# mfkiwl/conan-slam

Measured on AMD Instinct MI355X. Metric: ekf_update_steps_per_sec, higher is better.
Workload: dtype f32

## Files before the change

### conan_slam_amd/_capi.py

```python
from __future__ import annotations

import ctypes as C
import os
import re

_HERE = os.path.dirname(os.path.abspath(__file__))
LIB_PATH = os.path.join(_HERE, "lib", "libcslam_hip.so")
HEADER_PATH = os.path.join(_HERE, "..", "include", "cslam.h")

OK, ERR_BAD_ARG, ERR_CAPACITY, ERR_HIP, ERR_NO_DEVICE, ERR_ALLOC = 0, 1, 2, 3, 4, 5
FACTOR_OK, FACTOR_FALLBACK, FACTOR_ZEROED, FACTOR_SKIPPED, FACTOR_BAD_IDF, FACTOR_INTERNAL = 0, 1, 2, 4, 8, 16
FACTOR_HEADING_SKIPPED = 32
F32, F64 = 0, 1
Q_LOWER_CHOL_GAIN, Q_PREDICT_NM4, Q_REF_EXACT, Q_TEXTBOOK = 1, 2, 3, 0
STAGE_GATHER, STAGE_FACTOR, STAGE_GAIN, STAGE_DOWNDATE, N_STAGES = 0, 1, 2, 3, 4
STAGE_NAMES = ["gather", "factor", "gain", "downdate"]


class CslamError(RuntimeError):
    def __init__(self, code: int, msg: str):
        super().__init__(f"cslam status {code}: {msg}")
        self.code = code


BATCH_MC_SYMBOLS = ("cslam_ekf_batch_predict_each", "cslam_ekf_batch_get_poses")

LANDMARK_SYMBOLS = ("cslam_ekf_get_landmarks", "cslam_ekf_batch_get_landmarks")
_PROTOTYPES = {
    "cslam_ekf_get_landmarks": [C.c_void_p, C.c_int, C.c_int, C.c_void_p, C.c_void_p, C.c_void_p],
    "cslam_ekf_batch_get_landmarks": [C.c_void_p, C.c_int, C.c_int, C.c_void_p, C.c_void_p, C.c_void_p],
    "cslam_sim_batch_create": [C.c_void_p, C.c_int, C.c_int, C.POINTER(C.c_longlong), C.c_int, C.POINTER(C.c_void_p)],
    "cslam_sim_batch_destroy": [C.c_void_p],
    "cslam_sim_batch_scan": [C.c_void_p, C.c_void_p, C.c_double, C.c_void_p, C.c_longlong, C.POINTER(C.c_int),
                             C.POINTER(C.c_int), C.POINTER(C.c_int)],
    "cslam_sim_batch_get_scan": [C.c_void_p, C.c_int, C.c_void_p, C.c_void_p, C.c_void_p, C.c_void_p],
    "cslam_sim_batch_get_table": [C.c_void_p, C.c_void_p],
    "cslam_sim_batch_set_table": [C.c_void_p, C.c_void_p],
    "cslam_ekf_batch_update_scan": [C.c_void_p, C.c_void_p, C.c_void_p],
    "cslam_ekf_batch_augment_scan": [C.c_void_p, C.c_void_p, C.c_void_p],
}
SIM_BATCH_SYMBOLS = tuple(k for k in _PROTOTYPES if "sim_batch" in k or k.endswith("_scan"))


def declared_symbols(header_path: str = HEADER_PATH):
    text = open(header_path).read()
    text = re.sub(r"/\*.*?\*/", "", text, flags=re.S)
    return sorted(set(re.findall(r"\b(cslam_[a-z0-9_]+)\s*\(", text)))


_lib = None
hip_runtime_path = None


# ... 45 lines not shown
```

### conan_slam_amd/csrc/cslam_ekf.hip

```cpp
#include <hip/hip_runtime.h>

#include <algorithm>
#include <atomic>
#include <cfloat>
#include <cmath>
#include <cstdint>
#include <cstdlib>
#include <new>
#include <string>
#include <thread>
#include <vector>

#include "cslam_common.hpp"
#include "device_owners.hpp"
#include "ekf_kernels.hpp"
#include "ekf_kernels_fast.hpp"
#include "ekf_landmark_kernels.hpp"
#include "ekf_lookahead.hpp"
#include "ekf_pgemm_limbs.hpp"
#include "ekf_pose_kernels.hpp"
#include "host_linalg.hpp"

namespace cslam
{
// ... 18 lines not shown
        }
        else
        {
            j.idf_out[i - 2 * j.m] = j.idf[i - 2 * j.m];
        }
    }
    return true;
}
__global__ void __launch_bounds__(128) ekf_la_wide_f32(LaWideArgs a)
{
    if (la_wide_snapshot(a.snap))
    {
        return;
    }
    ekf_la_wide_body<1, 0>(a);
}
__global__ void __launch_bounds__(128) ekf_la_wide_f32_k64(LaWideArgs a)
{
    if (la_wide_snapshot(a.snap))
    {
        return;
    }
    ekf_la_wide_body<1, 64>(a);
}
}

using namespace cslam;

namespace
{

std::atomic<int>& g_engines = ::cslam::live_engines();

constexpr int    kStagingSlots = 64;
constexpr size_t kLdsBudget    = 150 * 1024;

struct EkfBase
{
    virtual ~EkfBase() {}
    int         dtype    = CSLAM_F32;
    int         fuse_f64 = 1;
    int         pgemm_limbs_req = -1, limbs_kmin_req = -1;
    int         xcd_queues_req = -1;
    int         device   = 0;
    int         quirks   = CSLAM_Q_REF_EXACT;
    int         nmax     = 0;
    int         ncap     = 0;
    int         ldp      = 0;
    int         n        = 3;
    int         sync_mode = 1;
    int         seq_defer     = 1;
    int         lower         = 0;
    int         pipeline      = 0;
    int         pgemm_spare   = 16;
    int         gather_corr_wide = 1;
    int         pgemm_wgs     = 0;
    int         lookahead     = -1;
    Stream      stream_own, stream_b_own, stream_f_own;
    hipStream_t stream   = nullptr;
    hipStream_t stream_b = nullptr;
    long long   la_windows = 0;
    long long   stage_launches = 0;

    virtual int init()                                                                        = 0;
    virtual int set_state(const void* X, int n, const void* P, int ldp)                        = 0;
    virtual int get_state(void* X, void* P, int ldp)                                           = 0;
    virtual int get_x(void* X, int cap)                                                        = 0;
    virtual int get_landmarks(int first, int count, void* x, void* pll, void* pvl)             = 0;
    virtual int trace(double* tr)                                                              = 0;
    virtual int predict(double v, double swa, const void* Q, double wb, double dt)             = 0;
    virtual int update(const void* Z, int m, const void* R, const int* idf, int batch, bool on_device) = 0;
    virtual int augment(const void* Z, int q, const void* R)                                   = 0;
    virtual int observe_heading(double phi, int use)                                           = 0;
    virtual int associate(const void* Z, int m, const void* R, double g1, double g2, int* idf_out, int* kind) = 0;
    virtual int factor_status(int* flags, int clear)                                           = 0;
    virtual int set_profiling(int on)                                                          = 0;
    virtual int get_stage_times(double* ms, int* launches)                                     = 0;
    virtual int debug_last_update(void* PHT, void* S, void* G, void* W1, void* V, int* k)      = 0;
    virtual int set_deferred(int max_cols)                                                     = 0;
    virtual int do_flush()                                                                     = 0;
    virtual int resolve_predict()                                                              = 0;
    virtual void set_fuse_predict(int on)                                                      = 0;
    virtual int sync_all()                                                                     = 0;
    virtual int la_drain()                                                                     = 0;
};
// ... 164 lines not shown
        {
            CSLAM_HIP_TRY(hipFuncSetAttribute(reinterpret_cast<const void*>(&ekf_factor_mfma_f64<64>),
                                              hipFuncAttributeMaxDynamicSharedMemorySize, 160 * 1024));
            CSLAM_HIP_TRY(hipFuncSetAttribute(reinterpret_cast<const void*>(&ekf_factor_mfma_f64<32>),
                                              hipFuncAttributeMaxDynamicSharedMemorySize, 160 * 1024));
            CSLAM_HIP_TRY(hipFuncSetAttribute(reinterpret_cast<const void*>(&ekf_downdate_f64<4>),
                                              hipFuncAttributeMaxDynamicSharedMemorySize, 160 * 1024));
            CSLAM_HIP_TRY(hipFuncSetAttribute(reinterpret_cast<const void*>(&ekf_downdate_f64<2>),
                                              hipFuncAttributeMaxDynamicSharedMemorySize, 160 * 1024));
        }
        CSLAM_TRY(dTicket.alloc_zeroed(2, stream));
        if (const char* sv = getenv("CSLAM_LA_K64"))
        {
            la_k64 = atoi(sv) ? 1 : 0;
        }
        if (const char* sv = getenv("CSLAM_LA_WG_SIGNAL"))
        {
            la_wg_signal = atoi(sv) ? 1 : 0;
        }
        if (const char* sv = getenv("CSLAM_LA_HOLD_WIDE"))
        {
            la_hold_wide = atoi(sv) ? 1 : 0;
        }
        if (const char* sv = getenv("CSLAM_PSYM_NT"))
        {
            psym_nt = atoi(sv) ? 1 : 0;
        }
        rc = ensure_k(64);
        if (rc)
        {
            return rc;
        }
        rc = ensure_w(128);
        if (rc)
        {
            return rc;
        }
        rc = ensure_m(64);
        if (rc)
        {
            return rc;
        }
        CSLAM_HIP_TRY(hipStreamSynchronize(stream));
        return CSLAM_OK;
    }

// ... 18 lines not shown
        if (cols <= wcap)
        {
            return CSLAM_OK;
        }
        int rc = flush();
        if (rc || (rc = sync_all()))
        {
            return rc;
        }
        int neww = round_up(std::max(cols, 2 * wcap), 8);
        DevBuf<T>   w1, y;
        DevBuf<int> sign;
        if ((rc = w1.alloc_zeroed((size_t)2 * ldp * neww, stream)) || (rc = y.alloc((size_t)std::max(kcap, 8) * neww)) ||
            (rc = sign.alloc_zeroed((size_t)2 * neww + 2, stream)))
        {
            return rc;
        }
        dW1   = std::move(w1);
        ws.dY = std::move(y);
        dSign = std::move(sign);
        hd_cols[0] = hd_cols[1] = 0;
        wcap      = neww;
        wcur      = 0;
        last_slot = nullptr;
        return CSLAM_OK;
    }

    int sync_all() override
    {
        int rc = use_device();
        if (rc)
        {
            return rc;
        }
        CSLAM_HIP_TRY(hipStreamSynchronize(stream));
        if (stream_b != stream)
        {
            CSLAM_HIP_TRY(hipStreamSynchronize(stream_b));
        }
        if (stream_f)
        {
            CSLAM_HIP_TRY(hipStreamSynchronize(stream_f));
        }
        inflight_mask = 0;
        return CSLAM_OK;
    }
// ... 39 lines not shown
        {
            CSLAM_HIP_TRY(hipEventRecord(ev_a2b.get(), stream));
            CSLAM_HIP_TRY(hipStreamWaitEvent(stream_b, ev_a2b.get(), 0));
        }
        if (hd_cols[wcur] > 0)
        {
            if ((rc = launch_negcol_fix(W, kp, stream_b)))
            {
                return rc;
            }
        }
        if ((rc = prof_begin(CSLAM_STAGE_DOWNDATE, stream_b)) || (rc = launch_downdate(W, kp, stream_b)) ||
            (rc = prof_end(CSLAM_STAGE_DOWNDATE, stream_b)))
        {
            return rc;
        }
        if (stream_b != stream)
        {
            CSLAM_HIP_TRY(hipEventRecord(ev_pgemm.get(), stream_b));
            inflight_mask |= 1u << wcur;
        }
        wcur ^= 1;
        kp = 0;
        if ((rc = own_region(wcur)))
        {
            return rc;
        }
        if (hd_cols[wcur] > 0)
        {
            if (stream_b != stream)
            {
                CSLAM_HIP_TRY(hipMemsetAsync(dSign.get() + (size_t)wcur * wcap, 0, (size_t)wcap * sizeof(int), stream));
                CSLAM_HIP_TRY(hipMemsetAsync(dSign.get() + (size_t)2 * wcap + wcur, 0, sizeof(int), stream));
            }
            hd_cols[wcur] = 0;
        }
        return CSLAM_OK;
    }

    int ensure_tiles_morton(int tiles, hipStream_t stream)
    {
        if (tilesM_built == tiles)
        {
            return CSLAM_OK;
        }

// ... 151 lines not shown
        *dZ   = reinterpret_cast<const T*>(ds);
        *dIdf = reinterpret_cast<const int*>(ds + zb);
        return CSLAM_OK;
    }

    int set_state(const void* X, int nn, const void* P, int ldph) override
    {
        if (!X || !P || nn < 3 || nn > ncap || ((nn - 3) & 1) || ldph < nn)
        {
            return fail(CSLAM_ERR_BAD_ARG, "set_state: bad n=%d (cap %d) or ldp=%d", nn, ncap, ldph);
        }
        int rc = sync_all();
        if (rc)
        {
            return rc;
        }
        CSLAM_HIP_TRY(hipMemcpyAsync(dX.get(), X, (size_t)nn * sizeof(T), hipMemcpyHostToDevice, stream));
        CSLAM_HIP_TRY(hipMemcpy2DAsync(dP.get(), (size_t)ldp * sizeof(T), P, (size_t)ldph * sizeof(T),
                                       (size_t)nn * sizeof(T), (size_t)nn, hipMemcpyHostToDevice, stream));
        CSLAM_HIP_TRY(hipMemcpyAsync(dPv.get(), dP.get(), (size_t)3 * ldp * sizeof(T), hipMemcpyDeviceToDevice,
                                     stream));
        kp        = 0;
        wcur      = 0;
        last_slot = nullptr;
        hd_cols[0] = hd_cols[1] = 0;
        CSLAM_HIP_TRY(hipMemsetAsync(dSign.get(), 0, ((size_t)2 * wcap + 2) * sizeof(int), stream));
        CSLAM_HIP_TRY(hipMemsetAsync(ws.dPHT.get(), 0, (size_t)ldp * kcap * sizeof(T), stream));
        CSLAM_HIP_TRY(hipMemsetAsync(dW1.get(), 0, (size_t)2 * ldp * wcap * sizeof(T), stream));
        CSLAM_HIP_TRY(hipStreamSynchronize(stream));
        n = nn;
        return CSLAM_OK;
    }

    int get_state(void* X, void* P, int ldph) override
    {
        if (ldph < n && P)
        {
            return fail(CSLAM_ERR_BAD_ARG, "get_state: ldp=%d < n=%d", ldph, n);
        }
        int rc = use_device();
        if (rc)
        {
            return rc;
        }
        if (P && (rc = flush_wait()))
        {
// ... 711 lines not shown
    {
        DevBuf<T>   S, G, Gt, V, t, U, M, sub, xloc;
        DevBuf<int> idloc;
    };
    struct LaSet
    {
        Event          ev_fb;
        Event          ev_raw;
        FactorOut      fo[2];
        DevBuf<T>      XL, PvL, PH, PvLb, Dbb;
        DevBuf<T>      Y;
        DevBuf<LaModel<T>> model;
        DevBuf<unsigned>   done;
        DevBuf<long long>  stamps;
        DevBuf<int>        idf_keep;
        DevBuf<T>          z_keep;
    };
    struct LaHeld
    {
        bool       valid = false;
        bool       k64   = false;
        unsigned   grid  = 0;
        LaWideArgs wa;
    };
    LaHeld      la_held;
    int         la_hold_wide = 1;
    LaUpd       la_q[2];
    int         la_n = 0;
    LaSet       la;
    bool        la_ready = false;
    hipStream_t stream_f = nullptr;
    DevBuf<T>   la_WR;
    int         la_kpad  = 0;
    int         la_cus = 0;
    unsigned    la_target = 0;
    unsigned    la_seq    = 0;
    unsigned    la_sig_add = 0;
    int         la_k64 = 1;
    int         la_wg_signal = 0;

    int         la_fused   = 1;
    const T *dbgS = nullptr, *dbgGt = nullptr, *dbgV = nullptr;

    int la_ensure(int kp_cols)
    {
        constexpr int KM = 2 * kLaMaxObs;
        if (!la_ready)
        {
            int lo = 0, hi = 0;
            CSLAM_HIP_TRY(hipDeviceGetStreamPriorityRange(&lo, &hi));
            Stream sf;
            LaSet  nl;
            int    rc = sf.create_with_priority(hipStreamNonBlocking, hi);
            if (rc || (rc = nl.ev_fb.create(hipEventDisableTiming)) || (rc = nl.ev_raw.create(hipEventDisableTiming)))
            {
                return rc;
            }
            CSLAM_HIP_TRY(hipFuncSetAttribute(reinterpret_cast<const void*>(&ekf_la_chain_kernel<T, 32>),
                                              hipFuncAttributeMaxDynamicSharedMemorySize, (int)la_chain_lds<T>(32)));
            CSLAM_HIP_TRY(hipFuncSetAttribute(reinterpret_cast<const void*>(&ekf_la_chain_kernel<T, 64>),
                                              hipFuncAttributeMaxDynamicSharedMemorySize, (int)la_chain_lds<T>(64)));
            CSLAM_TRY(nl.done.alloc_zeroed_blocking(768));
// ... 19 lines not shown
            }
            if (const char* fv = getenv("CSLAM_LA_FUSED"))
            {
                la_fused = atoi(fv) ? 1 : 0;
            }
            stream_f_own = std::move(sf);
            stream_f     = stream_f_own.get();
            la           = std::move(nl);
            la_cus       = 1;
            la_target    = 0;
            la_seq       = 0;
            la_ready     = true;
        }
        if (kp_cols > la_kpad)
        {
            CSLAM_HIP_TRY(hipStreamSynchronize(stream));
            CSLAM_HIP_TRY(hipStreamSynchronize(stream_f));
            const int kpad = round_up(std::max(kp_cols, 128), 64);
            DevBuf<T> wr;
            CSLAM_TRY(wr.alloc((size_t)2 * KM * kpad));
            la_WR   = std::move(wr);
            la_kpad = kpad;
        }
        return CSLAM_OK;
    }

    bool la_eligible(int m) const
    {
        const int k = 2 * m;
        const bool on = lookahead > 0 || (lookahead < 0 && sizeof(T) == 4 && n >= 7000 && g_engines.load() == 1);
        return on && !sync_mode && !pipeline && profiling != 1 && k > 16 && k <= 2 * kLaMaxObs && gather_corr_wide &&
               fuse_predict && (sizeof(T) == 4 || fuse_f64) && defer_max >= k + (la_n ? 2 * la_q[0].m : k) &&
               wcap >= k + (la_n ? 2 * la_q[0].m : k) && seq.count == 0 && hd_cols[0] == 0 && hd_cols[1] == 0 && n > 3 &&
               kp_call_limit == 0;
    }

    int la_launch_held_wide(const LaSnapJob* job)
    {
        if (!la_held.valid)
        {
            return CSLAM_OK;
        }
        if constexpr (std::is_same<T, float>::value)
        {
            int rc = use_device();
            if (rc)
            {
                return rc;
            }
            if (g_engines.load() > 1)
            {
                CSLAM_HIP_TRY(hipStreamWaitEvent(stream, la.ev_fb.get(), 0));
            }
            LaWideArgs& wa = la_held.wa;
            unsigned    g  = la_held.grid;
            if (job != nullptr)
            {
                wa.snap = *job;
                g += 1;
            }
            if (la_held.k64)
            {
                hipLaunchKernelGGL(ekf_la_wide_f32_k64, dim3(g), dim3(128), 0, stream, wa);
            }
            else
            {
                hipLaunchKernelGGL(ekf_la_wide_f32, dim3(g), dim3(128), 0, stream, wa);
            }
            CSLAM_HIP_TRY(hipGetLastError());
        }
        la_held.valid = false;
        return CSLAM_OK;
    }

    int la_enqueue(const T* dZ, const int* dIdf, int m, const T* R, bool on_device)
    {
        if (on_device && la_n == 0)
        {
            int rc = la_held.valid ? ensure_m(m) : CSLAM_OK;
            if (rc)
            {
                return rc;
            }
            if constexpr (std::is_same<T, float>::value)
// ... 206 lines not shown
            return rc;
        }
        const T* Wp = wbase(wcur);
        LaRowsArgs<T> ra;
        ra.X     = dX.get();
        ra.Pv    = dPv.get();
        ra.ldp   = ldp;
        ra.n     = n;
        ra.idf_a = ua.dIdf;
        ra.ra    = ka;
        ra.idf_b = nu == 2 ? ub.dIdf : ua.dIdf;
        ra.rb    = kb;
        ra.Wp    = Wp;
        ra.ldw   = ldp;
        ra.kp    = kp;
        ra.kpad  = la_kpad;
        ra.XL    = la.XL.get();
        ra.PvL   = la.PvL.get();
        ra.WR    = la_WR.get();
        ra.flags = dFlags.get();
        ra.idf_b_keep = hold ? la.idf_keep.get() : (int*)nullptr;
        ra.Z_b        = ub.dZ;
        ra.Z_b_keep   = hold ? la.z_keep.get() : (T*)nullptr;
        hipLaunchKernelGGL(ekf_la_rows_kernel<T>, dim3(ka + kb), dim3(128), 0, stream, ra);
        LaPrepArgs<T> pa;
        pa.P       = dP.get();
        pa.ldp     = ldp;
        pa.n       = n;
        pa.lower   = lower;
        pa.X       = dX.get();
        pa.Pv      = dPv.get();
        pa.idf_a   = ua.dIdf;
        pa.idf_b   = nu == 2 ? ub.dIdf : ua.dIdf;
        pa.ra      = ka;
        pa.rb      = kb;
        pa.pp_a    = ua.pp;
        pa.XL      = la.XL.get();
        pa.PvL     = la.PvL.get();
        pa.WR      = la_WR.get();
        pa.kp      = kp;
        pa.kpad    = la_kpad;
        pa.sub_a   = la.fo[0].sub.get();
        pa.PH      = la.PH.get();
        pa.Dbb     = la.Dbb.get();
        pa.PvLb    = la.PvLb.get();
        pa.model_a = la.model.get();
        pa.xloc_a  = la.fo[0].xloc.get();
        pa.idloc   = la.fo[0].idloc.get();
        const int  k8f      = round_up(kp, 8);
        const bool pg_signal = !la_wg_signal && !safe && kp > 0 && seq.count == 0 && sizeof(T) == 4 && k8f <= 128 && lower && ldp < 32768 &&
                               !limbs_take(k8f) && stream_b == stream && hd_cols[wcur] == 0;
        pa.done    = pg_signal ? (unsigned*)nullptr : la.done.get();
        hipLaunchKernelGGL(ekf_la_blocks_kernel<T>, dim3(n_blocks), dim3(64), 0, stream, pa);
        CSLAM_HIP_TRY(hipGetLastError());
        if (safe)
        {
            CSLAM_HIP_TRY(hipEventRecord(la.ev_raw.get(), stream));
            CSLAM_HIP_TRY(hipStreamWaitEvent(stream_f, la.ev_raw.get(), 0));
            if ((rc = launch_chain()))
            {
                return rc;
            }
        }
        la_target += n_blocks;
        la_sig_add = pg_signal ? n_blocks : 0u;
        rc         = flush();
        if (la_sig_add != 0)
        {
            const unsigned add = la_sig_add;
            la_sig_add         = 0;
            hipLaunchKernelGGL(ekf_la_signal_kernel, dim3(1), dim3(64), 0, stream, la.done.get(), add);
        }
        if (rc)
        {
            return rc;
        }
// ... 23 lines not shown
                wa.mb      = nu == 2 ? ub.m : 0;
                wa.valid_a = ua.pp.valid;
                wa.valid_b = nu == 2 ? ub.pp.valid : 0;
                wa.w_a     = ua.pp.w;
                wa.w_b     = nu == 2 ? ub.pp.w : 0;
                wa.model_a = la.model.get();
                wa.model_b = la.model.get() + 1;
                wa.Gt_a    = la.fo[0].Gt.get();
                wa.u_a     = la.fo[0].U.get();
                wa.M_a     = la.fo[0].M.get();
                wa.sub_a   = la.fo[0].sub.get();
                wa.Gt_b    = la.fo[1].Gt.get();
                wa.u_b     = la.fo[1].U.get();
                wa.M_b     = la.fo[1].M.get();
                wa.sub_b   = la.fo[1].sub.get();
                wa.Y_b     = la.Y.get();
                wa.W1a     = wbase(wcur) + (size_t)kp * ldp;
                wa.W1b     = wa.W1a + (size_t)ka * ldp;
                wa.ldw     = ldp;
                wa.wv_out  = ws.dWv.get();
                wa.snap    = LaSnapJob{nullptr, nullptr, nullptr, nullptr, 0};
                la_held.wa    = wa;
                la_held.k64   = la_k64 && ua.m == 32 && (nu == 1 || ub.m == 32);
                la_held.grid  = (unsigned)(round_up(n, kTile) / 32);
                la_held.valid = true;
                if (!hold && (rc = la_launch_held_wide(nullptr)))
                {
                    return rc;
                }
                last_slot = nullptr;
                last_k    = 0;
                kp += ka + kb;
                sub_valid = false;
            }
        }
        if (!fused && ((rc = la_wide(ua, la.fo[0], la.ev_fb.get())) || (nu == 2 && (rc = la_wide(ub, la.fo[1],
                                                                                                 nullptr)))))
        {
            return rc;
        }
        pp = held;
        la_windows++;
        if (la.stamps.get() && la_windows == 300)
        {
            long long h[32];
            CSLAM_HIP_TRY(hipStreamSynchronize(stream));
// ... 783 lines not shown

int cslam_ekf_set_pgemm_workgroups(cslam_ekf_t h, int workgroups)
{
    CSLAM_NEED(h);
    if (workgroups < 0)
    {
        return fail(CSLAM_ERR_BAD_ARG, "set_pgemm_workgroups: negative");
    }
    B(h)->pgemm_wgs = workgroups;
    return CSLAM_OK;
}

int cslam_ekf_lookahead_windows(cslam_ekf_t h, long long* windows)
{
    CSLAM_NEED(h);
    if (!windows)
    {
        return fail(CSLAM_ERR_BAD_ARG, "lookahead_windows: null");
    }
    *windows = B(h)->la_windows;
    return CSLAM_OK;
}

int cslam_ekf_stage_launches(cslam_ekf_t h, long long* launches)
{
    CSLAM_NEED(h);
    if (!launches)
    {
        return fail(CSLAM_ERR_BAD_ARG, "stage_launches: null");
    }
    *launches = B(h)->stage_launches;
    return CSLAM_OK;
}

int cslam_ekf_get_streams(cslam_ekf_t h, void** chain_stream, void** pgemm_stream)
{
    CSLAM_NEED(h);
    if (chain_stream)
    {
        *chain_stream = reinterpret_cast<void*>(B(h)->stream);
    }
    if (pgemm_stream)
    {
        *pgemm_stream = reinterpret_cast<void*>(B(h)->stream_b);
    }
    return CSLAM_OK;
// ... 109 lines not shown
```

### conan_slam_amd/csrc/ekf_lookahead.hpp

```cpp
#pragma once

#include <hip/hip_runtime.h>

#include "ekf_kernels.hpp"
#include "ekf_kernels_fast.hpp"

namespace cslam
{

constexpr int kLaMaxObs = 32;

__device__ inline int la_row(const int* __restrict__ idf, int s, int n)
{
    return 3 + 2 * clamp_idf(idf[s >> 1], n) - 2 + (s & 1);
}

template <typename T>
struct LaRowsArgs
{
    const T* X;
    const T* Pv;
    int      ldp, n;
    const int* idf_a;
    int        ra;
// ... 316 lines not shown
            out[2 * tid + 1] = v1;
        }
        if (type == 2 && tid < 3)
        {
            a.PvLb[s * 3 + tid] = s_e3[tid];
        }
    }
    if (a.done == nullptr)
    {
        return;
    }
    __builtin_amdgcn_fence(__ATOMIC_RELEASE, "agent");
    __syncthreads();
    if (tid == 0)
    {
        atomicAdd(a.done + 16 * (blockIdx.x & 15u), 1u);
    }
}

template <typename T>
__global__ void __launch_bounds__(64) ekf_la_blocks_kernel(LaPrepArgs<T> a)
{
    ekf_la_blocks_body<T>(a);
}

template <typename T>
struct LaCarryArgs
{
    int n, m_a, m_b;
    const int* idf_b;
    PredictArgs<T> pp_b;
    const T *PH, *Dbb, *PvLb, *XLb;
    const LaModel<T>* model_a;
    const T *Gt_a, *u_a, *M_a, *sub_a;
    T*          sub_b;
    T*          xloc_b;
    LaModel<T>* model_b;
    T*          Y_b;
};

template <typename T>
inline size_t la_carry_lds()
{
    constexpr int KM = 2 * kLaMaxObs, LD = KM + 4, LB = 3 + KM + 1;
    return ((size_t)KM * LD + (size_t)(3 + KM) * LB + kLaMaxObs * 10 + (3 + KM) + 4 * KM + 3 * KM) * sizeof(T) + 64;
}
// ... 404 lines not shown
    const int *  idf_a, *idf_b;
    int          ma, mb;
    int          valid_a, valid_b, w_a, w_b;
    const LaModel<float>*model_a, *model_b;
    const float *Gt_a, *u_a, *M_a, *sub_a;
    const float *Gt_b, *u_b, *M_b, *sub_b, *Y_b;
    float *      W1a, *W1b;
    int          ldw;
    float*       wv_out;
    const unsigned* chain_done;
    unsigned        seq;
    unsigned long long timeout;
    int*            flags;
    long long*      stamps;
    long long*      wg_times;
    LaSnapJob       snap;
};

__device__ __forceinline__ int la_q_of(int t, int r, int lh)
{
    return 32 * t + (r & 3) + 8 * (r >> 2) + 4 * lh;
}

template <int PAIRS = 1, int KFIX = 0>
__device__ __forceinline__ void ekf_la_wide_body(const LaWideArgs& a)
{
    __shared__ __attribute__((aligned(16))) float s_G[2][4 * 1024];
    __shared__ __attribute__((aligned(16))) float s_Y[4 * 1024];
    __shared__ __attribute__((aligned(16))) float s_model[2][512];
    __shared__ __attribute__((aligned(16))) float s_u[2][256];
    __shared__ __attribute__((aligned(16))) float s_M[2][256];
    __shared__ int   s_fx[2][kLaMaxObs];
    __shared__ float s_sum_all[PAIRS][4][32];
    const int tid = threadIdx.x, wave = __builtin_amdgcn_readfirstlane(tid >> 6), lane = tid & 63, lj = lane & 31, lh = lane >> 5;
    const int wv = wave & 1, pr = wave >> 1;
    float (*s_sum)[32] = s_sum_all[pr];
    const int row0 = (blockIdx.x * PAIRS + pr) * 32;
    const int row  = row0 + lj;
    const int rowc = row < a.n ? row : a.n - 1;
    const int ka = KFIX ? KFIX : 2 * a.ma, kb = KFIX ? KFIX : 2 * a.mb;
    int       stamp_i = 0;
    auto      stamp   = [&]() {
        if (a.stamps != nullptr && blockIdx.x == (gridDim.x >> 1) && tid == 0)
        {
            a.stamps[stamp_i++] = (long long)__builtin_amdgcn_s_memrealtime();
        }
    };
    stamp();
    if constexpr (PAIRS == 2)
// ... 183 lines not shown
    };
    auto store_w1 = [&](float* W, int k, bool last) {
#pragma unroll
        for (int r = 0; r < 16; r++)
        {
            const int c = la_q_of(wv, r, lh);
            if (c < k)
            {
                if (row < 3)
                {
                    if (last)
                    {
                        a.wv_out[(size_t)row * k + c] = w1[r];
                    }
                    W[(size_t)c * a.ldw + row] = 0.f;
                }
                else
                {
                    W[(size_t)c * a.ldw + row] = w1[r];
                }
            }
        }
    };
    using U0 = std::integral_constant<int, 0>;
    using U1 = std::integral_constant<int, 1>;

    if (a.valid_a && row >= 3 && row - 3 < a.w_a)
    {
        float o0, o1, o2;
        predict_stripe_col<float>(s_model[0][0], s_model[0][1], pv0, pv1, pv2, &o0, &o1, &o2);
        pv0 = o0, pv1 = o1, pv2 = o2;
    }
    build_own(U0{}, ka, a.sub_a);
    share();
    stamp();
    gain(U0{}, ka);
    stamp();
    store_w1(a.W1a, ka, a.nu == 1);
    const float* pred_last = s_model[0];
    if (a.nu == 2)
    {
        __syncthreads();
#pragma unroll
        for (int r = 0; r < 16; r++)
        {
            own[r] = (row >= 3) ? w1[r] : 0.f;
        }
        share();
        const float xs = s_sum[0][lj], xm0 = s_sum[1][lj], xm1 = s_sum[2][lj], xm2 = s_sum[3][lj];
        if (row >= 3)
        {
            x += xs;
            pv0 -= xm0, pv1 -= xm1, pv2 -= xm2;
        }
        stamp();
        if (a.valid_b && row >= 3 && row - 3 < a.w_b)
        {
            float o0, o1, o2;
            predict_stripe_col<float>(s_model[1][0], s_model[1][1], pv0, pv1, pv2, &o0, &o1, &o2);
            pv0 = o0, pv1 = o1, pv2 = o2;
        }
// ... 24 lines not shown
                    c0 = __builtin_amdgcn_mfma_f32_32x32x2f32(y[i], full[i], c0, 0, 0, 0);
                }
            }
            if (row >= 3)
            {
#pragma unroll
                for (int r = 0; r < 16; r++)
                {
                    own[r] -= c0[r] + c1[r];
                }
            }
        }
        stamp();
        __syncthreads();
        dma(a.Gt_b, kb * kb, s_G[1]);
        xch = s_G[0] + pr * 2048;
        share();
        __builtin_amdgcn_s_waitcnt(0x0F70);
        __syncthreads();
        stamp();
        gain(U1{}, kb);
        stamp();
        store_w1(a.W1b, kb, true);
        pred_last = s_model[1];
    }
    __syncthreads();
    stamp();
    if constexpr (PAIRS == 2)
    {
        if (a.wg_times != nullptr && tid == 0)
        {
            a.wg_times[2 * blockIdx.x + 1] = (long long)__builtin_amdgcn_s_memrealtime();
        }
    }
    if (wv == 0 && lh == 0 && row < a.n)
    {
        const float xs = s_sum[0][lj], xm0 = s_sum[1][lj], xm1 = s_sum[2][lj], xm2 = s_sum[3][lj];
        if (row >= 3)
        {
            a.X[row]                        = x + xs;
            a.Pv[(size_t)0 * a.ldp + row] = pv0 - xm0;
            a.Pv[(size_t)1 * a.ldp + row] = pv1 - xm1;
            a.Pv[(size_t)2 * a.ldp + row] = pv2 - xm2;
        }
        else
        {
// ... 242 lines not shown
```

### conan_slam_amd/ekf.py

```python
from __future__ import annotations

import ctypes as C

import numpy as np

from . import _capi
from ._capi import (F32, F64, Q_REF_EXACT, Q_TEXTBOOK, check)


def _vp(a: np.ndarray):
    return a.ctypes.data_as(C.c_void_p)


class EKF:
    def __init__(self, max_landmarks: int, dtype=np.float32, device: int = -1, quirks: int = Q_REF_EXACT,
                 sync_mode: bool = True):
        self.dtype = np.dtype(dtype)
        if self.dtype not in (np.dtype(np.float32), np.dtype(np.float64)):
            raise ValueError("dtype must be float32 or float64")
        self._L = _capi.lib()
        self._h = C.c_void_p(None)
        code = F32 if self.dtype == np.float32 else F64
        check(self._L.cslam_ekf_create(C.c_int(max_landmarks), C.c_int(code), C.c_int(device), C.c_int(quirks),
                                       C.byref(self._h)))
# ... 71 lines not shown
    P = property(get_p)

    def trace(self) -> float:
        t = C.c_double(0.0)
        check(self._L.cslam_ekf_trace(self._h, C.byref(t)))
        return t.value

    def synchronize(self):
        check(self._L.cslam_ekf_synchronize(self._h))

    def lookahead_windows(self) -> int:
        w = C.c_longlong(0)
        check(self._L.cslam_ekf_lookahead_windows(self._h, C.byref(w)))
        return w.value

    def streams(self):
        a, b = C.c_void_p(None), C.c_void_p(None)
        check(self._L.cslam_ekf_get_streams(self._h, C.byref(a), C.byref(b)))
        return a.value or 0, b.value or 0

    def stage_launches(self) -> int:
        w = C.c_longlong(0)
        check(self._L.cslam_ekf_stage_launches(self._h, C.byref(w)))
        return w.value

    def landmarks(self, first: int = 1, count: int = None):
        if count is None:
            count = max((self.n - 3) // 2 - first + 1, 0)
        x = np.empty((count, 2), dtype=self.dtype)
        pll = np.empty((count, 4), dtype=self.dtype)
        pvl = np.empty((count, 6), dtype=self.dtype)
        check(self._L.cslam_ekf_get_landmarks(self._h, int(first), int(count), _vp(x), _vp(pll), _vp(pvl)))
        return x, pll.reshape(count, 2, 2).transpose(0, 2, 1).copy(), pvl.reshape(count, 2, 3).transpose(0, 2, 1).copy()

    def factor_status(self, clear: bool = False) -> int:
        f = C.c_int(0)
        check(self._L.cslam_ekf_factor_status(self._h, C.byref(f), C.c_int(1 if clear else 0)))
        return f.value

    def predict(self, v, swa, Q, wb, dt):
        Q = self._mat22(Q)
        check(self._L.cslam_ekf_predict(self._h, C.c_double(float(v)), C.c_double(float(swa)), _vp(Q),
                                        C.c_double(float(wb)), C.c_double(float(dt))))

    def update(self, Z, R, idf, batch: bool = False):
        Z = np.asarray(Z, dtype=self.dtype)
# ... 231 lines not shown
```

### include/cslam.h

```cpp
#ifndef CSLAM_H
#define CSLAM_H

#ifdef __cplusplus
extern "C" {
#endif

#define CSLAM_VERSION 100

#define CSLAM_OK 0
#define CSLAM_ERR_BAD_ARG 1
#define CSLAM_ERR_CAPACITY 2
#define CSLAM_ERR_HIP 3
#define CSLAM_ERR_NO_DEVICE 4
#define CSLAM_ERR_ALLOC 5
#define CSLAM_FACTOR_OK 0
#define CSLAM_FACTOR_FALLBACK 1
#define CSLAM_FACTOR_ZEROED 2
#define CSLAM_FACTOR_SKIPPED 4
#define CSLAM_FACTOR_INTERNAL 16
#define CSLAM_FACTOR_BAD_IDF 8
#define CSLAM_FACTOR_HEADING_SKIPPED 32

#define CSLAM_F32 0
#define CSLAM_F64 1
// ... 31 lines not shown
int cslam_ekf_factor_status(cslam_ekf_t h, int* flags, int clear);

int cslam_ekf_predict(cslam_ekf_t h, double v, double swa, const void* Q, double wb, double dt);

int cslam_ekf_update(cslam_ekf_t h, const void* Z, int m, const void* R, const int* idf, int batch);

int cslam_ekf_update_device(cslam_ekf_t h, const void* dZ, int m, const void* R, const int* d_idf, int batch);

int cslam_ekf_augment(cslam_ekf_t h, const void* Z, int q, const void* R);

int cslam_ekf_observe_heading(cslam_ekf_t h, double phi, int use_heading);

int cslam_ekf_associate(cslam_ekf_t h, const void* Z, int m, const void* R, double gate1, double gate2, int* idf_out,
                        int* kind_out);

int cslam_ekf_set_deferred(cslam_ekf_t h, int max_pending_columns);
int cslam_ekf_flush(cslam_ekf_t h);

int cslam_ekf_get_streams(cslam_ekf_t h, void** chain_stream, void** pgemm_stream);

int cslam_ekf_lookahead_windows(cslam_ekf_t h, long long* windows);

int cslam_ekf_stage_launches(cslam_ekf_t h, long long* launches);

int cslam_ekf_set_pgemm_workgroups(cslam_ekf_t h, int workgroups);

int cslam_ekf_run_many(cslam_ekf_t* handles, int count, int steps, const double* v, const double* swa, const void* Q,
                       double wb, double dt, const void* const* dZ, const int* const* d_idf, int m, const void* R,
                       int batch);

typedef struct cslam_ekf_batch* cslam_ekf_batch_t;
int cslam_ekf_batch_create(int instances, int n_landmarks, int device, int quirks, cslam_ekf_batch_t* out);
int cslam_ekf_batch_destroy(cslam_ekf_batch_t h);
int cslam_ekf_batch_set_state(cslam_ekf_batch_t h, int instance, const float* X, int n, const float* P, int ldp);
int cslam_ekf_batch_get_state(cslam_ekf_batch_t h, int instance, float* X, float* P, int ldp);
int cslam_ekf_batch_run(cslam_ekf_batch_t h, int steps, const double* v, const double* swa, const float* Q, double wb,
                        double dt, const float* const* dZ, const int* const* d_idf, int m, const float* R);
int cslam_ekf_batch_flush(cslam_ekf_batch_t h);
int cslam_ekf_batch_synchronize(cslam_ekf_batch_t h);
int cslam_ekf_batch_trace(cslam_ekf_batch_t h, double* traces );
int cslam_ekf_batch_factor_status(cslam_ekf_batch_t h, int* flags );
int cslam_ekf_batch_info(cslam_ekf_batch_t h, int* instances, int* n, long long* windows);
int cslam_ekf_batch_set_profiling(cslam_ekf_batch_t h, int every);
int cslam_ekf_batch_get_pgemm_time(cslam_ekf_batch_t h, double* ms_sum, int* launches);

int cslam_ekf_batch_create_capacity(int instances, int max_landmarks, int n_landmarks, int device, int quirks,
// ... 93 lines not shown
```

Before: 13610.

## Mirror lookahead gain rows into a transposed buffer to skip the rows kernel

The wide k64 lookahead kernel now also writes its W1 gain columns into a row-major mirror buffer (WT). On the next window, a new blocks kernel reads that mirror to compute the pending rank-k correction dot products itself, so the separate ekf_la_rows_kernel launch is skipped. This removes one kernel launch per lookahead step and its global round trip. In exchange the wide kernel does extra stores, a larger-LDS 256-thread blocks kernel runs, and there are new state-tracking conditions for when the mirror is valid.

```diff
diff --git a/conan_slam_amd/_capi.py b/conan_slam_amd/_capi.py
--- a/conan_slam_amd/_capi.py
+++ b/conan_slam_amd/_capi.py
@@ -29,6 +29,7 @@
 _PROTOTYPES = {
     "cslam_ekf_get_landmarks": [C.c_void_p, C.c_int, C.c_int, C.c_void_p, C.c_void_p, C.c_void_p],
     "cslam_ekf_batch_get_landmarks": [C.c_void_p, C.c_int, C.c_int, C.c_void_p, C.c_void_p, C.c_void_p],
+    "cslam_ekf_rows_launches": [C.c_void_p, C.POINTER(C.c_longlong)],
     "cslam_sim_batch_create": [C.c_void_p, C.c_int, C.c_int, C.POINTER(C.c_longlong), C.c_int, C.POINTER(C.c_void_p)],
     "cslam_sim_batch_destroy": [C.c_void_p],
     "cslam_sim_batch_scan": [C.c_void_p, C.c_void_p, C.c_double, C.c_void_p, C.c_longlong, C.POINTER(C.c_int),
diff --git a/conan_slam_amd/csrc/cslam_ekf.hip b/conan_slam_amd/csrc/cslam_ekf.hip
--- a/conan_slam_amd/csrc/cslam_ekf.hip
+++ b/conan_slam_amd/csrc/cslam_ekf.hip
@@ -64,6 +64,20 @@
         return;
     }
     ekf_la_wide_body<1, 64>(a);
+}
+
+__global__ void __launch_bounds__(128) ekf_la_wide_f32_k64m(LaWideArgs a, float* WT)
+{
+    if (la_wide_snapshot(a.snap))
+    {
+        return;
+    }
+    ekf_la_wide_body<1, 64, 1>(a, WT);
+}
+
+__global__ void __launch_bounds__(256) ekf_la_blocks_mirror_kernel(LaPrepArgs<float> a, LaMirrorArgs mi)
+{
+    ekf_la_blocks_mirror_body(a, mi);
 }
 }
 
@@ -103,6 +117,7 @@
     hipStream_t stream_b = nullptr;
     long long   la_windows = 0;
     long long   stage_launches = 0;
+    long long   rows_launches = 0;
 
     virtual int init()                                                                        = 0;
     virtual int set_state(const void* X, int n, const void* P, int ldp)                        = 0;
@@ -313,6 +328,10 @@
         {
             la_hold_wide = atoi(sv) ? 1 : 0;
         }
+        if (const char* sv = getenv("CSLAM_LA_MIRROR"))
+        {
+            la_mirror = atoi(sv) ? 1 : 0;
+        }
         if (const char* sv = getenv("CSLAM_PSYM_NT"))
         {
             psym_nt = atoi(sv) ? 1 : 0;
@@ -377,6 +396,7 @@
         hd_cols[0] = hd_cols[1] = 0;
         wcap      = neww;
         wcur      = 0;
+        la_mirror_cols = 0;
         last_slot = nullptr;
         return CSLAM_OK;
     }
@@ -462,6 +482,7 @@
         }
         wcur ^= 1;
         kp = 0;
+        la_mirror_cols = 0;
         if ((rc = own_region(wcur)))
         {
             return rc;
@@ -659,6 +680,7 @@
                                      stream));
         kp        = 0;
         wcur      = 0;
+        la_mirror_cols = 0;
         last_slot = nullptr;
         hd_cols[0] = hd_cols[1] = 0;
         CSLAM_HIP_TRY(hipMemsetAsync(dSign.get(), 0, ((size_t)2 * wcap + 2) * sizeof(int), stream));
@@ -1416,6 +1438,7 @@
         bool       k64   = false;
         unsigned   grid  = 0;
         LaWideArgs wa;
+        float*     wt = nullptr;
     };
     LaHeld      la_held;
     int         la_hold_wide = 1;
@@ -1432,6 +1455,11 @@
     unsigned    la_sig_add = 0;
     int         la_k64 = 1;
     int         la_wg_signal = 0;
+    DevBuf<float> la_WT;
+    int           la_wt_rows     = 0;
+    int           la_mirror_cols = 0;
+    int           la_mirror_n    = 0;
+    int           la_mirror      = 1;
 
     int         la_fused   = 1;
     const T *dbgS = nullptr, *dbgGt = nullptr, *dbgV = nullptr;
@@ -1497,6 +1525,17 @@
             la_WR   = std::move(wr);
             la_kpad = kpad;
         }
+        if (la_mirror && std::is_same<T, float>::value && round_up(n, kTile) > la_wt_rows)
+        {
+            CSLAM_HIP_TRY(hipStreamSynchronize(stream));
+            CSLAM_HIP_TRY(hipStreamSynchronize(stream_f));
+            const int     rows = round_up(n, kTile);
+            DevBuf<float> wt;
+            CSLAM_TRY(wt.alloc((size_t)rows * 128));
+            la_WT          = std::move(wt);
+            la_wt_rows     = rows;
+            la_mirror_cols = 0;
+        }
         return CSLAM_OK;
     }
 
@@ -1534,7 +1573,11 @@
                 wa.snap = *job;
                 g += 1;
             }
-            if (la_held.k64)
+            if (la_held.k64 && la_held.wt != nullptr)
+            {
+                hipLaunchKernelGGL(ekf_la_wide_f32_k64m, dim3(g), dim3(128), 0, stream, wa, la_held.wt);
+            }
+            else if (la_held.k64)
             {
                 hipLaunchKernelGGL(ekf_la_wide_f32_k64, dim3(g), dim3(128), 0, stream, wa);
             }
@@ -1787,7 +1830,16 @@
         ra.idf_b_keep = hold ? la.idf_keep.get() : (int*)nullptr;
         ra.Z_b        = ub.dZ;
         ra.Z_b_keep   = hold ? la.z_keep.get() : (T*)nullptr;
-        hipLaunchKernelGGL(ekf_la_rows_kernel<T>, dim3(ka + kb), dim3(128), 0, stream, ra);
+        bool use_mirror = false;
+        if constexpr (std::is_same<T, float>::value)
+        {
+            use_mirror = la_mirror && (kp == 0 || (la_mirror_cols == kp && la_mirror_n == n && kp <= 128 && kp % 4 == 0));
+        }
+        if (!use_mirror)
+        {
+            hipLaunchKernelGGL(ekf_la_rows_kernel<T>, dim3(ka + kb), dim3(128), 0, stream, ra);
+            rows_launches++;
+        }
         LaPrepArgs<T> pa;
         pa.P       = dP.get();
         pa.ldp     = ldp;
@@ -1816,7 +1868,24 @@
         const bool pg_signal = !la_wg_signal && !safe && kp > 0 && seq.count == 0 && sizeof(T) == 4 && k8f <= 128 && lower && ldp < 32768 &&
                                !limbs_take(k8f) && stream_b == stream && hd_cols[wcur] == 0;
         pa.done    = pg_signal ? (unsigned*)nullptr : la.done.get();
-        hipLaunchKernelGGL(ekf_la_blocks_kernel<T>, dim3(n_blocks), dim3(64), 0, stream, pa);
+        if constexpr (std::is_same<T, float>::value)
+        {
+            if (use_mirror)
+            {
+                LaMirrorArgs mi;
+                mi.WT         = la_WT.get();
+                mi.XLb        = la.XL.get() + ka;
+                mi.flags      = dFlags.get();
+                mi.idf_b_keep = ra.idf_b_keep;
+                mi.Z_b        = ra.Z_b;
+                mi.Z_b_keep   = ra.Z_b_keep;
+                hipLaunchKernelGGL(ekf_la_blocks_mirror_kernel, dim3(n_blocks), dim3(256), 0, stream, pa, mi);
+            }
+        }
+        if (!use_mirror)
+        {
+            hipLaunchKernelGGL(ekf_la_blocks_kernel<T>, dim3(n_blocks), dim3(64), 0, stream, pa);
+        }
         CSLAM_HIP_TRY(hipGetLastError());
         if (safe)
         {
@@ -1886,6 +1955,9 @@
                 wa.snap    = LaSnapJob{nullptr, nullptr, nullptr, nullptr, 0};
                 la_held.wa    = wa;
                 la_held.k64   = la_k64 && ua.m == 32 && (nu == 1 || ub.m == 32);
+                la_held.wt     = (la_mirror && la_held.k64 && kp == 0) ? la_WT.get() : nullptr;
+                la_mirror_cols = la_held.wt ? ka + kb : 0;
+                la_mirror_n    = n;
                 la_held.grid  = (unsigned)(round_up(n, kTile) / 32);
                 la_held.valid = true;
                 if (!hold && (rc = la_launch_held_wide(nullptr)))
@@ -2715,6 +2787,17 @@
     return CSLAM_OK;
 }
 
+int cslam_ekf_rows_launches(cslam_ekf_t h, long long* launches)
+{
+    CSLAM_NEED(h);
+    if (!launches)
+    {
+        return fail(CSLAM_ERR_BAD_ARG, "rows_launches: null");
+    }
+    *launches = B(h)->rows_launches;
+    return CSLAM_OK;
+}
+
 int cslam_ekf_stage_launches(cslam_ekf_t h, long long* launches)
 {
     CSLAM_NEED(h);
diff --git a/conan_slam_amd/csrc/ekf_lookahead.hpp b/conan_slam_amd/csrc/ekf_lookahead.hpp
--- a/conan_slam_amd/csrc/ekf_lookahead.hpp
+++ b/conan_slam_amd/csrc/ekf_lookahead.hpp
@@ -362,6 +362,266 @@
 __global__ void __launch_bounds__(64) ekf_la_blocks_kernel(LaPrepArgs<T> a)
 {
     ekf_la_blocks_body<T>(a);
+}
+
+struct LaMirrorArgs
+{
+    const float* WT;
+    float*       XLb;
+    int*         flags;
+    int*         idf_b_keep;
+    const float* Z_b;
+    float*       Z_b_keep;
+};
+
+constexpr int kLaWtLd = 128 + 4;
+
+__device__ __forceinline__ void ekf_la_blocks_mirror_body(const LaPrepArgs<float>& a, const LaMirrorArgs& mi)
+{
+    using T = float;
+    __shared__ __attribute__((aligned(16))) T s_wt[2 * kLaMaxObs * kLaWtLd];
+    __shared__ __attribute__((aligned(16))) T wrow[128];
+    __shared__ T s_xl[3 + 2 * kLaMaxObs];
+    __shared__ T s_coef[kLaMaxObs * 10];
+    __shared__ T s_pvv[9], s_g[2], s_e3[3];
+    __shared__ T s_d[2 * kLaMaxObs];
+    __shared__ T s_e[2 * kLaMaxObs * 3];
+    const int tid = threadIdx.x;
+    const int ra = a.ra, rb = a.rb, ma = ra >> 1;
+    int       b    = blockIdx.x;
+    int       type = 0, s = b;
+    if (b >= 3)
+    {
+        b -= 3;
+        type = (b < ra) ? 1 : ((b < ra + rb) ? 2 : 3);
+        s    = (type == 1) ? b : ((type == 2) ? b - ra : b - ra - rb);
+    }
+    const int* idf_r = (type <= 1) ? a.idf_a : a.idf_b;
+    const int* idf_c = (type == 3) ? a.idf_b : a.idf_a;
+    const int  nc    = (type == 3) ? rb : ra;
+    const int  pc = tid & 31, c0 = tid >> 5;
+    auto       row_of = [&](int id, int slot) { return 3 + 2 * clamp_idf(id, a.n) - 2 + (slot & 1); };
+    int cs[8], idc[8];
+#pragma unroll
+    for (int i = 0; i < 8; i++)
+    {
+        cs[i]  = min(c0 + 8 * i, nc - 1);
+        idc[i] = idf_c[cs[i] >> 1];
+    }
+    const int id_r = idf_r[s >> 1];
+    const int ct = min(tid, nc - 1), at = min(tid, ra - 1);
+    int       id_p = 1, id_a = 1;
+    T         warm[4] = {(T)0, (T)0, (T)0, (T)0};
+    if (tid < 64)
+    {
+        id_p = idf_c[ct >> 1];
+        id_a = a.idf_a[at >> 1];
+        warm[0] = a.X[0], warm[1] = a.Pv[0], warm[2] = a.Pv[(size_t)a.ldp], warm[3] = a.Pv[(size_t)2 * a.ldp];
+    }
+    __builtin_amdgcn_s_waitcnt(0x0F70);
+    const int  row    = row_of(id_r, s);
+    const int  erow   = row_of(id_a, at), prow = row_of(id_p, ct);
+    const bool mirror = a.kp > 0 && type != 0;
+    float4     w0, w1, w2, w3, w4, w5, w6, w7, wown;
+    w0 = w1 = w2 = w3 = w4 = w5 = w6 = w7 = wown = make_float4(0.f, 0.f, 0.f, 0.f);
+    if (mirror)
+    {
+        w0   = *reinterpret_cast<const float4*>(mi.WT + (size_t)row_of(idc[0], cs[0]) * 128 + 4 * pc);
+        w1   = *reinterpret_cast<const float4*>(mi.WT + (size_t)row_of(idc[1], cs[1]) * 128 + 4 * pc);
+        w2   = *reinterpret_cast<const float4*>(mi.WT + (size_t)row_of(idc[2], cs[2]) * 128 + 4 * pc);
+        w3   = *reinterpret_cast<const float4*>(mi.WT + (size_t)row_of(idc[3], cs[3]) * 128 + 4 * pc);
+        w4   = *reinterpret_cast<const float4*>(mi.WT + (size_t)row_of(idc[4], cs[4]) * 128 + 4 * pc);
+        w5   = *reinterpret_cast<const float4*>(mi.WT + (size_t)row_of(idc[5], cs[5]) * 128 + 4 * pc);
+        w6   = *reinterpret_cast<const float4*>(mi.WT + (size_t)row_of(idc[6], cs[6]) * 128 + 4 * pc);
+        w7   = *reinterpret_cast<const float4*>(mi.WT + (size_t)row_of(idc[7], cs[7]) * 128 + 4 * pc);
+        wown = *reinterpret_cast<const float4*>(mi.WT + (size_t)row * 128 + 4 * pc);
+    }
+    T   pcell = (T)0, xa = (T)0, xr = (T)0;
+    T   e3[3] = {(T)0, (T)0, (T)0}, ee[3] = {(T)0, (T)0, (T)0};
+    if (tid < 64)
+    {
+        pcell = p_sym<T>(a.P, a.ldp, row, prow, a.lower);
+        xa    = a.X[erow];
+        xr    = a.X[row];
+#pragma unroll
+        for (int c = 0; c < 3; c++)
+        {
+            e3[c] = a.Pv[(size_t)c * a.ldp + row];
+            ee[c] = a.Pv[(size_t)c * a.ldp + erow];
+        }
+    }
+    const bool keep = type == 2 && mi.idf_b_keep != nullptr;
+    T          zb   = (T)0;
+    int        ib   = 0;
+    if (keep)
+    {
+        zb = mi.Z_b[s];
+        ib = a.idf_b[s >> 1];
+    }
+    if (mirror)
+    {
+        float4* dst = reinterpret_cast<float4*>(&s_wt[c0 * kLaWtLd + 4 * pc]);
+        dst[0 * 2 * kLaWtLd] = w0;
+        dst[1 * 2 * kLaWtLd] = w1;
+        dst[2 * 2 * kLaWtLd] = w2;
+        dst[3 * 2 * kLaWtLd] = w3;
+        dst[4 * 2 * kLaWtLd] = w4;
+        dst[5 * 2 * kLaWtLd] = w5;
+        dst[6 * 2 * kLaWtLd] = w6;
+        dst[7 * 2 * kLaWtLd] = w7;
+        *reinterpret_cast<float4*>(&wrow[4 * pc]) = wown;
+    }
+    if (type != 0 && type != 3 && tid == 0 && (id_r < 1 || id_r > ((a.n - 3) >> 1)))
+    {
+        atomicOr(&mi.flags[0], kFlagBadIdf);
+    }
+    if (tid < ra)
+    {
+        s_xl[3 + tid] = xa;
+    }
+    asm volatile("" : : "v"(warm[0]), "v"(warm[1]), "v"(warm[2]), "v"(warm[3]));
+    if (tid == 0)
+    {
+        T pose_in[3] = {a.X[0], a.X[1], a.X[2]}, pvv_in[9], pose[3], g[2], pvv[9];
+        for (int e = 0; e < 9; e++)
+        {
+            pvv_in[e] = a.Pv[(size_t)(e / 3) * a.ldp + (e % 3)];
+        }
+        la_predict_pose<T>(a.pp_a, pose_in, pvv_in, pose, g, pvv);
+        s_xl[0] = pose[0], s_xl[1] = pose[1], s_xl[2] = pose[2];
+        s_g[0] = g[0], s_g[1] = g[1];
+        for (int e = 0; e < 9; e++)
+        {
+            s_pvv[e] = pvv[e];
+        }
+        if (type != 0)
+        {
+            la_predict_row<T>(a.pp_a, g[0], g[1], row, e3);
+            s_e3[0] = e3[0], s_e3[1] = e3[1], s_e3[2] = e3[2];
+        }
+    }
+    __syncthreads();
+    if (tid < ma)
+    {
+        T   v[2];
+        int fx;
+        observe_model_pose<T>(s_xl, 3 + ra, tid + 1, (T)0, (T)0, s_xl[0], s_xl[1], s_xl[2], &s_coef[tid * 10], v, &fx);
+    }
+    if (type == 0)
+    {
+        if (tid < ra)
+        {
+            la_predict_row<T>(a.pp_a, s_g[0], s_g[1], erow, ee);
+            s_e[tid * 3 + 0] = ee[0], s_e[tid * 3 + 1] = ee[1], s_e[tid * 3 + 2] = ee[2];
+        }
+    }
+    else if (tid < nc)
+    {
+        const T* wc  = s_wt + tid * kLaWtLd;
+        T        dot = (T)0;
+        int      q   = 0;
+#pragma unroll 4
+        for (; q + 4 <= a.kp; q += 4)
+        {
+            const float4 v = *reinterpret_cast<const float4*>(wc + q);
+            const float4 w = *reinterpret_cast<const float4*>(&wrow[q]);
+            dot += w.x * v.x;
+            dot += w.y * v.y;
+            dot += w.z * v.z;
+            dot += w.w * v.w;
+        }
+        for (; q < a.kp; q++)
+        {
+            dot += wrow[q] * wc[q];
+        }
+        s_d[tid] = pcell - dot;
+    }
+    __syncthreads();
+    if (type == 0)
+    {
+        const int r = s;
+        if (tid < ma)
+        {
+            T v0, v1;
+            la_pht_pair<T>(&s_coef[tid * 10], s_pvv[r], s_pvv[r + 3], s_pvv[r + 6], s_e[(2 * tid) * 3 + r],
+                           s_e[(2 * tid + 1) * 3 + r], &v0, &v1);
+            a.sub_a[r * ra + 2 * tid]     = v0;
+            a.sub_a[r * ra + 2 * tid + 1] = v1;
+        }
+        if (r == 0)
+        {
+            LaModel<T>& mo = *a.model_a;
+            if (tid == 0)
+            {
+                mo.g02 = s_g[0];
+                mo.g12 = s_g[1];
+            }
+            if (tid < 3)
+            {
+                mo.pose[tid] = s_xl[tid];
+            }
+            if (tid < 9)
+            {
+                mo.pvv[tid] = s_pvv[tid];
+            }
+            for (int e = tid; e < ma * 10; e += 256)
+            {
+                mo.coef[e] = s_coef[e];
+            }
+            for (int e = tid; e < 3 + ra; e += 256)
+            {
+                a.xloc_a[e] = s_xl[e];
+            }
+            if (tid < kLaMaxObs)
+            {
+                a.idloc[tid] = tid + 1;
+            }
+        }
+    }
+    else if (type == 3)
+    {
+        if (tid < nc)
+        {
+            a.Dbb[(size_t)s * rb + tid] = s_d[tid];
+        }
+    }
+    else
+    {
+        if (tid < ma)
+        {
+            T v0, v1;
+            la_pht_pair<T>(&s_coef[tid * 10], s_e3[0], s_e3[1], s_e3[2], s_d[2 * tid], s_d[2 * tid + 1], &v0, &v1);
+            T* out           = (type == 1) ? (a.sub_a + (size_t)(3 + s) * ra) : (a.PH + (size_t)s * ra);
+            out[2 * tid]     = v0;
+            out[2 * tid + 1] = v1;
+        }
+        if (type == 2 && tid < 3)
+        {
+            a.PvLb[s * 3 + tid] = s_e3[tid];
+        }
+    }
+    if (type == 2 && tid == 0)
+    {
+        mi.XLb[s] = xr;
+        if (keep)
+        {
+            mi.Z_b_keep[s] = zb;
+            if ((s & 1) == 0)
+            {
+                mi.idf_b_keep[s >> 1] = ib;
+            }
+        }
+    }
+    if (a.done == nullptr)
+    {
+        return;
+    }
+    __builtin_amdgcn_fence(__ATOMIC_RELEASE, "agent");
+    __syncthreads();
+    if (tid == 0)
+    {
+        atomicAdd(a.done + 16 * (blockIdx.x & 15u), 1u);
+    }
 }
 
 template <typename T>
@@ -812,9 +1072,10 @@
     return 32 * t + (r & 3) + 8 * (r >> 2) + 4 * lh;
 }
 
-template <int PAIRS = 1, int KFIX = 0>
-__device__ __forceinline__ void ekf_la_wide_body(const LaWideArgs& a)
-{
+template <int PAIRS = 1, int KFIX = 0, int MIRROR = 0>
+__device__ __forceinline__ void ekf_la_wide_body(const LaWideArgs& a, float* wt = nullptr)
+{
+    static_assert(!MIRROR || (PAIRS == 1 && KFIX == 64), "the mirror belongs to the single filter's k = 64 kernel");
     __shared__ __attribute__((aligned(16))) float s_G[2][4 * 1024];
     __shared__ __attribute__((aligned(16))) float s_Y[4 * 1024];
     __shared__ __attribute__((aligned(16))) float s_model[2][512];
@@ -1044,6 +1305,15 @@
             }
         }
     };
+    auto store_wt = [&](int q0) {
+        float* dst = wt + (size_t)row * 128 + q0 + 32 * wv + 4 * lh;
+#pragma unroll
+        for (int g = 0; g < 4; g++)
+        {
+            const float4 v = make_float4(w1[4 * g], w1[4 * g + 1], w1[4 * g + 2], w1[4 * g + 3]);
+            *reinterpret_cast<float4*>(dst + 8 * g) = (row < 3) ? make_float4(0.f, 0.f, 0.f, 0.f) : v;
+        }
+    };
     using U0 = std::integral_constant<int, 0>;
     using U1 = std::integral_constant<int, 1>;
 
@@ -1059,6 +1329,10 @@
     gain(U0{}, ka);
     stamp();
     store_w1(a.W1a, ka, a.nu == 1);
+    if constexpr (MIRROR)
+    {
+        store_wt(0);
+    }
     const float* pred_last = s_model[0];
     if (a.nu == 2)
     {
@@ -1129,6 +1403,10 @@
         gain(U1{}, kb);
         stamp();
         store_w1(a.W1b, kb, true);
+        if constexpr (MIRROR)
+        {
+            store_wt(64);
+        }
         pred_last = s_model[1];
     }
     __syncthreads();
diff --git a/conan_slam_amd/ekf.py b/conan_slam_amd/ekf.py
--- a/conan_slam_amd/ekf.py
+++ b/conan_slam_amd/ekf.py
@@ -117,6 +117,11 @@
     def stage_launches(self) -> int:
         w = C.c_longlong(0)
         check(self._L.cslam_ekf_stage_launches(self._h, C.byref(w)))
+        return w.value
+
+    def rows_launches(self) -> int:
+        w = C.c_longlong(0)
+        check(self._L.cslam_ekf_rows_launches(self._h, C.byref(w)))
         return w.value
 
     def landmarks(self, first: int = 1, count: int = None):
diff --git a/include/cslam.h b/include/cslam.h
--- a/include/cslam.h
+++ b/include/cslam.h
@@ -77,6 +77,8 @@
 int cslam_ekf_lookahead_windows(cslam_ekf_t h, long long* windows);
 
 int cslam_ekf_stage_launches(cslam_ekf_t h, long long* launches);
+
+int cslam_ekf_rows_launches(cslam_ekf_t h, long long* launches);
 
 int cslam_ekf_set_pgemm_workgroups(cslam_ekf_t h, int workgroups);
 
```

Result: faster. 13800, median of 6 (+1.4%).
